# spectralDNS/mpiFFT4py

Hardware: AMD Instinct MI355X
Metric: 3D R2C+C2R pairs/sec, 1024^3 fp64 slab (higher is better)
Workload: dtype f64; 1 GPU; 1024^3 fp64 slab R2C forward+inverse, device-resident, 1 rank(s); gpus_visible=1

## Files before the change

### mpifft4py_amd/csrc/core.hip

```cpp
#include <algorithm>
#include <cstdarg>
#include <type_traits>
#include <cstdio>
#include <cstdlib>
#include <map>
#include <mutex>
#include <unordered_map>
#include <tuple>
#include "mfft_internal.h"
#include "fft_nlz.h"

namespace mfft {

static thread_local std::string g_err;

int set_error(int code, const char* fmt, ...) {
  char buf[1024];
  va_list ap;
  va_start(ap, fmt);
  vsnprintf(buf, sizeof buf, fmt, ap);
  va_end(ap);
  g_err = buf;
  return code;
}
const char* last_error() { return g_err.c_str(); }

std::vector<KernelEntry>& kernel_registry() {
  static std::vector<KernelEntry> reg;
  return reg;
}

constexpr int OP_BITS = 5, BUILD_BITS = 3, FAMILY_BITS = 6;
static_assert(2 * (unsigned)Op::TopFlag <= (1u << OP_BITS) && (unsigned)Op::Band < (unsigned)Op::Limited, "Op does not fit its key field");
static_assert((unsigned)Build::Last < (1u << BUILD_BITS), "Build does not fit its key field");
static_assert((unsigned)FAM_NLZ < (1u << FAMILY_BITS), "Family does not fit its key field");
static uint64_t kernel_key(int family, int n, int prec, int inv, Op op, Build build) {
  uint64_t k = (unsigned)n;
  k = k << FAMILY_BITS | (uint64_t)family;
  k = k << OP_BITS | (uint64_t)op;
  k = k << BUILD_BITS | (uint64_t)build;
  return k << 2 | (uint64_t)(inv << 1 | prec);
}

const KernelEntry* find_kernel(int family, int n, int prec, int inv, Op op, Build build) {
  static std::unordered_map<uint64_t, const KernelEntry*> index;
  static std::once_flag once;
  std::call_once(once, [] {
// ... 328 lines not shown
    P.bhat = static_cast<const cx<T>*>(bhat);
    P.n = a.n;
  }
  P.in = a.in;
  P.out = a.out;
  P.tw = static_cast<const cx<T>*>(tw);
  P.rtw = static_cast<const cx<T>*>(rtw);
  P.in_stride = a.in_stride;
  P.out_stride = a.out_stride;
  P.nrows = a.nrows;
  P.valid = a.valid > 0 ? a.valid : a.n / 2 + 1;
  P.scale = (T)a.scale;
  if constexpr (std::is_same<PT, RealParams<T>>::value) set_zsplit(P, a.zs);
  return launch_rows(e, P, a.nrows, e->tile, s);
}

static int c2r_mlds_mode() {
  static const int m = getenv("MFFT_C2R_MLDS") ? atoi(getenv("MFFT_C2R_MLDS")) : 1;
  return m;
}
static bool c2r_mlds_take(int n, int prec, bool limited) {
  const int m = c2r_mlds_mode();
  if (m <= 0) return false;
  if (m == 2) return true;
  if (m == 3) return limited;
  const int c = n / 2;
  if (c == 1000 || c == 2000) return prec == MFFT_SINGLE;
  if (c == 1536) return limited && prec == MFFT_SINGLE;
  if (c == 2048) return !limited && prec == MFFT_DOUBLE;
  return true;
// ... 6 lines not shown
    if (const KernelEntry* em = find_kernel(fam, a.n, a.prec, 1, op, Build::LdsMirrors)) e = em;
  const int64_t real_stride = fam == FAM_R2C ? a.in_stride : a.out_stride;
  if (a.zs.nchunk && (!e || real_stride % 2 != 0)) return set_error(MFFT_ERR_UNSUPPORTED, "no z-chunked real kernel of length %d", a.n);
  if (!e && limited) return set_error(MFFT_ERR_UNSUPPORTED, "no column-limited real kernel of length %d", a.n);
  if (!e || (real_stride % 2 != 0 && !limited)) {
    const bool r2c = fam == FAM_R2C;
    const bool half = a.n % 2 == 0 && a.n >= 4 && real_stride % 2 == 0;
    e = find_chirpz(half ? (r2c ? FAM_R2CZH : FAM_C2RZH) : (r2c ? FAM_R2CZ : FAM_C2RZ), half ? a.n / 2 : a.n, a.prec, r2c ? 0 : 1);
    if (!e && !big_length_ok(a.n)) return set_error(MFFT_ERR_UNSUPPORTED, "no kernel for a real transform of length %d", a.n);
  } else if (real_stride % 2 != 0) {
    return set_error(MFFT_ERR_UNSUPPORTED, "real row stride %lld must be even", (long long)real_stride);
  }
  *out = e;
  return 0;
}
static int launch_real(int fam, const RealArgs& a, hipStream_t s) {
  const KernelEntry* e = nullptr;
  MFFT_TRY(select_real(fam, a, &e));
  if (!e) return big_real(fam == FAM_C2R, a, s);
  void *tw = nullptr, *rtw = nullptr, *chirp = nullptr, *bhat = nullptr;
  MFFT_TRY(prepare_kernel(e, &tw));
  if (e->family != fam) {
    const bool half = e->family == FAM_R2CZH || e->family == FAM_C2RZH;
    MFFT_TRY(chirpz_tables(half ? a.n / 2 : a.n, e->n, a.prec, &chirp, &bhat));
    if (half) MFFT_TRY(real_twiddles(a.n, a.prec, &rtw));
    return by_prec(a.prec, [&](auto t) { return launch_real_t<decltype(t), RealParamsZ<decltype(t)>>(e, a, tw, rtw, s, chirp, bhat); });
  }
  MFFT_TRY(real_twiddles(a.n, a.prec, &rtw));
  return by_prec(a.prec, [&](auto t) { return launch_real_t<decltype(t)>(e, a, tw, rtw, s); });
}

int launch_r2c(const RealArgs& a, hipStream_t s) { return launch_real(FAM_R2C, a, s); }
// ... 208 lines not shown
```

### mpifft4py_amd/csrc/fft_kernels.h

```cpp
#pragma once
#include "fft_core.h"

#if defined(__HIPCC__)
#define MFFT_D __device__ __forceinline__
#define MFFT_BARRIER() __syncthreads()
#if defined(__HIP_DEVICE_COMPILE__)
#define MFFT_OPAQUE(x) asm volatile("" : "+v"(x))
#else
#define MFFT_OPAQUE(x) ((void)0)
#endif
template <class S, bool ORIGIN = false> MFFT_D int row_thread_index(int tid) {
  int j = tid % S::TPT;
  if constexpr (::mfft::launder_plan<S>()) {
#if MFFT_LAUNDER_MODE == 1
    MFFT_OPAQUE(j);
#elif MFFT_LAUNDER_MODE == 4
    if constexpr (ORIGIN) MFFT_OPAQUE(j);
#endif
  }
  return j;
}
#else
#define MFFT_OPAQUE(x) ((void)0)
template <class S, bool ORIGIN = false> inline int row_thread_index(int tid) { return tid % S::TPT; }
// ... 114 lines not shown
};

template <typename T>
struct RealParams {
  const void* in;
  void* out;
  const cx<T>* tw;
  const cx<T>* rtw;
  i64 in_stride, out_stride;
  i64 nrows;
  int valid;
  T scale;
  ZSplit zs;
  i64 row0;
};

template <int PD> MFFT_HD int padpos(int pos) {
  if constexpr (PD > 0) return pos + pos / PD;
  else return pos;
}
template <int N, int PD> constexpr int padded_len() { return PD > 0 ? N + N / PD + 1 : N; }
template <int PD> struct PadSlot {
  MFFT_D int operator()(int pos) const { return padpos<PD>(pos); }
};

template <typename T, class Slot>
struct XchFull {
  cx<T>* buf;
  Slot slot;
  template <class S, int P>
// ... 447 lines not shown
      for (int k = 0; k < S::E; ++k) {
        cx<T> x = scale(v[k], P.scale);
        x = INV ? swapri(x) : x;
        if constexpr (CHUNK && !INV) {
          bool ok;
          const i64 o = zsplit_off(P.zs, crow, j + k * S::TPT, &ok);
          if (ok) P.out[o] = x;
        } else {
          op[j + k * S::TPT] = x;
        }
      }
    }
  }
};

template <class S, typename T, int ROWS, bool TWLDS, bool LIMIT = false, bool CHUNK = false, bool SPLIT = false, bool WP = false>
struct R2CFft {
  typedef typename RowXch<SPLIT, T, PadSlot<S::R(0)>>::elem XE;
  static constexpr int M = S::N;
  static constexpr int RPW = WP ? 64 / S::TPT : 1;
  static_assert(!WP || (S::TPT < 64 && 64 % S::TPT != 0 && ROWS % (64 / S::TPT) == 0), "wave-packed rows: whole waves of rows");
  static constexpr int THREADS = WP ? ROWS / RPW * 64 : S::TPT * ROWS;
  static constexpr int PD = S::R(0);
  static constexpr int PLEN = padded_len<M, PD>();
  static constexpr int TW_BYTES = TWLDS ? (int)(S::TW * sizeof(cx<T>)) : 0;
  static constexpr int XCH_BYTES = (int)(PLEN * ROWS * sizeof(XE));
  static constexpr int LDS_BYTES = TW_BYTES + XCH_BYTES;

  static MFFT_D void body(const RealParams<T>& P, int bid, int tid, char* lds) {
    cx<T>* ltw = reinterpret_cast<cx<T>*>(lds);
    int rl, j, lane0 = 0;
    bool dup = false;
    if constexpr (WP) {
      const int lane = tid & 63;
      int lr = lane / S::TPT;
      dup = lr >= RPW;
      if (dup) lr = RPW - 1;
      lane0 = lr * S::TPT;
      j = dup ? lane - RPW * S::TPT : lane - lane0;
#if MFFT_LAUNDER_MODE == 1
      if constexpr (S::E % 15 == 0) MFFT_OPAQUE(j);
#endif
      rl = (tid >> 6) * RPW + lr;
    } else {
      rl = tid / S::TPT;
      j = row_thread_index<S>(tid);
    }
    XE* xch = reinterpret_cast<XE*>(lds + TW_BYTES) + rl * PLEN;
    const i64 row = (i64)bid * ROWS + rl;
    const bool inrange = row < P.nrows;
    const bool active = inrange && !dup;
    const cx<T>* ip =
        reinterpret_cast<const cx<T>*>(static_cast<const T*>(P.in) + (inrange ? row : P.nrows - 1) * P.in_stride);
    cx<T>* op = static_cast<cx<T>*>(P.out) + row * P.out_stride;

    cx<T> v[S::E];
#pragma unroll
    for (int k = 0; k < S::E; ++k) v[k] = ip[j + k * S::TPT];
    if constexpr (TWLDS && S::NP > 1) {
      stage_twiddles<S, T>(ltw, P.tw, tid, THREADS);
      MFFT_BARRIER();
    }
    typename RowXch<SPLIT, T, PadSlot<PD>>::type xc{xch, PadSlot<PD>{}};
    if constexpr (TWLDS) run_passes<S, 0, T>(v, j, (const cx<T>*)ltw, xc);
    else run_passes<S, 0, T>(v, j, P.tw, xc);

    const T half = (T)0.5;
    auto put = [&](int pos, cx<T> val) {
      if constexpr (CHUNK) {
// ... 5 lines not shown
      }
    };
    auto emit_w = [&](int pos, cx<T> zk, cx<T> zpartner, cx<T> w) {
      if (pos == 0) {
        put(0, mk<T>((zk.x + zk.y) * P.scale, (T)0));
        if (!LIMIT || M < P.valid) put(M, mk<T>((zk.x - zk.y) * P.scale, (T)0));
      } else if (!LIMIT || pos < P.valid) {
        const cx<T> zm = conj(zpartner);
        const cx<T> e = scale(zk + zm, half);
        const cx<T> o = mul_mi(scale(zk - zm, half));
        put(pos, scale(e + w * o, P.scale));
      }
    };
    auto emit = [&](int pos, cx<T> zk, cx<T> zpartner) { emit_w(pos, zk, zpartner, P.rtw[pos]); };
    constexpr bool SHFL = WP || (S::TPT <= 64 && (64 % S::TPT) == 0);
    if constexpr (SHFL) {
      const int src = WP ? lane0 + (j == 0 ? 0 : S::TPT - j) : (tid & 63) - j + ((S::TPT - j) & (S::TPT - 1));
      constexpr bool RTW_EARLY = S::E * (int)sizeof(cx<T>) <= 128;
      cx<T> rt[RTW_EARLY ? S::E : 1];
      if constexpr (RTW_EARLY) {
#pragma unroll
        for (int k = 0; k < S::E; ++k) rt[k] = P.rtw[j + k * S::TPT];
      }
#pragma unroll
      for (int k = 0; k < S::E; ++k) {
        const cx<T> give = v[S::E - 1 - k];
        cx<T> pm = mk<T>(wave_shfl(give.x, src), wave_shfl(give.y, src));
        if (j == 0) pm = v[(S::E - k) % S::E];
        if constexpr (RTW_EARLY) {
          if (active) emit_w(j + k * S::TPT, v[k], pm, rt[k]);
        } else
// ... 32 lines not shown
#pragma unroll
      for (int k = 0; k < S::E; ++k) xc.put(j + k * S::TPT, v[k]);
      MFFT_BARRIER();
      if (active) {
#pragma unroll
        for (int k = 0; k < S::E; ++k) {
          const int pos = j + k * S::TPT;
          emit(pos, v[k], xc.get(pos == 0 ? 0 : M - pos));
        }
      }
    }
  }
};

template <class S, typename T, int ROWS, bool TWLDS, bool LIMIT = false, bool CHUNK = false, bool SPLIT = false, bool WP = false,
          bool MLDS = false>
struct C2RFft {
  typedef typename RowXch<SPLIT, T, PadSlot<S::R(0)>>::elem XE;
  static constexpr int M = S::N;
  static constexpr int RPW = WP ? 64 / S::TPT : 1;
  static_assert(!WP || (S::TPT < 64 && 64 % S::TPT != 0 && ROWS % (64 / S::TPT) == 0), "wave-packed rows: whole waves of rows");
  static constexpr int THREADS = WP ? ROWS / RPW * 64 : S::TPT * ROWS;
  static constexpr int PD = S::R(0);
  static constexpr int PLEN = padded_len<M, PD>();
  static constexpr int TW_BYTES = TWLDS ? (int)(S::TW * sizeof(cx<T>)) : 0;
  static constexpr int XCH_BYTES = S::NP > 1 ? (int)(PLEN * ROWS * sizeof(XE)) : 0;
  static constexpr int LDS_BYTES = TW_BYTES + XCH_BYTES;

  static MFFT_D void body(const RealParams<T>& P, int bid, int tid, char* lds) {
    cx<T>* ltw = reinterpret_cast<cx<T>*>(lds);
    int rl, j, lane0 = 0;
    bool dup = false;
    if constexpr (WP) {
      const int lane = tid & 63;
      int lr = lane / S::TPT;
      dup = lr >= RPW;
      if (dup) lr = RPW - 1;
      lane0 = lr * S::TPT;
      j = dup ? lane - RPW * S::TPT : lane - lane0;
      if constexpr (S::E % 15 == 0) MFFT_OPAQUE(j);
      rl = (tid >> 6) * RPW + lr;
    } else {
      rl = tid / S::TPT;
      j = row_thread_index<S, true>(tid);
    }
    XE* xch = reinterpret_cast<XE*>(lds + TW_BYTES) + rl * PLEN;
    const i64 row = (i64)bid * ROWS + rl;
    const bool inrange = row < P.nrows;
    const bool active = inrange && !dup;
    const cx<T>* ip = static_cast<const cx<T>*>(P.in) + (inrange ? row : P.nrows - 1) * P.in_stride;
    cx<T>* op = reinterpret_cast<cx<T>*>(static_cast<T*>(P.out) + row * P.out_stride);

    const i64 crow = P.row0 + (inrange ? row : P.nrows - 1);
    auto bin = [&](int pos) -> cx<T> {
      if constexpr (CHUNK) {
        bool ok;
        const i64 o = zsplit_off(P.zs, crow, pos, &ok);
        const cx<T> x = static_cast<const cx<T>*>(P.in)[ok ? o : (i64)0];
        if constexpr (sizeof(T) == 4) return keep_bits(x, ok);
        else return ok ? x : mk<T>((T)0, (T)0);
      } else {
        return ip[pos];
      }
    };
    cx<T> v[S::E];
    constexpr bool SHFL = WP || (S::TPT <= 64 && (64 % S::TPT) == 0);
    if constexpr (SHFL) {
      static_assert(S::E % 2 == 0, "register pairing needs an even number of values per thread");
#pragma unroll
      for (int k = 0; k < S::E; ++k) {
        const int pos = j + k * S::TPT;
        if constexpr (LIMIT && sizeof(T) == 4) {
          const bool ok = pos < P.valid;
          v[k] = keep_bits(bin(ok ? pos : 0), ok);
        } else if constexpr (LIMIT) {
          v[k] = mk<T>((T)0, (T)0);
          if (pos < P.valid) v[k] = bin(pos);
        } else {
          v[k] = bin(pos);
        }
      }
      cx<T> carry = mk<T>((T)0, (T)0);
// ... 20 lines not shown
        if constexpr (WP || S::E % 7 != 0) {
          pm1 = mk<T>(wave_shfl(give1.x, src), wave_shfl(give1.y, src));
          pm2 = mk<T>(wave_shfl(give2.x, src), wave_shfl(give2.y, src));
        } else {
          pm1 = mk<T>(WAVE_SHFL_DIRECT(give1.x, src), WAVE_SHFL_DIRECT(give1.y, src));
          pm2 = mk<T>(WAVE_SHFL_DIRECT(give2.x, src), WAVE_SHFL_DIRECT(give2.y, src));
        }
        carry = b;
        v[k] = prepass(a, pm1, j + k * S::TPT);
        v[kp] = prepass(b, pm2, j + kp * S::TPT);
        if constexpr (S::E % 15 == 0) {
          if (k % 3 == 2) MFFT_SCHED_FENCE();
        }
      }
    } else if constexpr (MLDS && S::NP > 1) {
#pragma unroll
      for (int k = 0; k < S::E; ++k) {
        const int pos = j + k * S::TPT;
        if constexpr (LIMIT) {
          const bool ok = pos < P.valid;
          v[k] = keep_bits(bin(ok ? pos : 0), ok);
        } else {
          v[k] = bin(pos);
        }
      }
      cx<T> xM = mk<T>((T)0, (T)0);
      if (j == 0 && (!LIMIT || M < P.valid)) xM = bin(M);
      auto prepass = [&](cx<T> xk, cx<T> pm, int pos) {
        cx<T> xm = conj(pm);
        if (pos == 0) {
// ... 85 lines not shown
```

### mpifft4py_amd/csrc/mfft_internal.h

```cpp
#pragma once
#include <hip/hip_runtime.h>
#include <stdint.h>
#include <string>
#include <vector>
#include "../../include/mpifft4py_amd.h"
#include "registry.h"

namespace mfft {

int set_error(int code, const char* fmt, ...) __attribute__((format(printf, 2, 3)));
const char* last_error();

#define MFFT_HIP(call)                                                                   \
  do {                                                                                   \
    hipError_t e_ = (call);                                                              \
    if (e_ != hipSuccess)                                                                \
      return ::mfft::set_error(MFFT_ERR_HIP, "%s failed: %s (%s:%d)", #call,             \
                               hipGetErrorString(e_), __FILE__, __LINE__);               \
  } while (0)

#define MFFT_TRY(call)                  \
  do {                                  \
    int rc_ = (call);                   \
    if (rc_ != 0) return rc_;           \
// ... 53 lines not shown
  int64_t in_stride = 0, out_stride = 0, nrows = 0;
  double scale = 1.0;
  ZSplitArgs zs;
};
int launch_row(const RowArgs& a, hipStream_t s);

struct RealArgs {
  const void* in = nullptr;
  void* out = nullptr;
  int n = 0;
  int prec = MFFT_DOUBLE;
  int64_t in_stride = 0, out_stride = 0, nrows = 0;
  double scale = 1.0;
  int valid = 0;
  ZSplitArgs zs;
};
int launch_r2c(const RealArgs& a, hipStream_t s);
int launch_c2r(const RealArgs& a, hipStream_t s);

struct NlzArgs {
  const void* a[3] = {nullptr, nullptr, nullptr};
  const void* b[3] = {nullptr, nullptr, nullptr};
  void* out[3] = {nullptr, nullptr, nullptr};
  int n = 0;
  int prec = MFFT_DOUBLE;
  int64_t in_stride = 0, out_stride = 0, nrows = 0;
  int valid = 0;
  int valid_in = 0;
  double scale = 1.0;
};
bool nlz_supported(int64_t n, int prec);
int launch_nlz(const NlzArgs& a, hipStream_t s);

// ... 32 lines not shown
```

### mpifft4py_amd/csrc/plan_create.hip

```cpp
#include "plan_impl.h"

using namespace mfft;

#ifndef MFFT_DEFAULT_COMM_CUS
#define MFFT_DEFAULT_COMM_CUS 0
#endif

mfft_plan_s::~mfft_plan_s() {
  for (Buf* b : {&work[0], &work[1], &work[2], &work3, &nlw[0], &nlw[1], &nlx, &nly, &nlr, &pcomp})
    if (b->p) (void)(b->arena ? wfree(b->p) : dev_free(b->p));
  if (mask) (void)hipFree(mask);
  if (band_tiles) (void)hipFree(band_tiles);
  for (auto& t : timers) {
    for (auto& e : t.pending) { (void)hipEventDestroy(e.first); (void)hipEventDestroy(e.second); }
    for (auto& e : t.pool) { (void)hipEventDestroy(e.first); (void)hipEventDestroy(e.second); }
  }
  drop_graphs();
  for (hipEvent_t e : ev_compute) (void)hipEventDestroy(e);
  for (hipEvent_t e : ev_comm) (void)hipEventDestroy(e);
  for (hipEvent_t e : ev2_compute) (void)hipEventDestroy(e);
  for (hipEvent_t e : ev2_comm) (void)hipEventDestroy(e);
  if (cstream) { big_release_stream(cstream); (void)hipStreamDestroy(cstream); }
  if (stream) { big_release_stream(stream); (void)hipStreamDestroy(stream); }
}
// ... 287 lines not shown
  if (!p || !key || !value) return set_error(MFFT_ERR_INVALID, "null argument");
  const std::string k(key);
  if (k == "pruned_route") *value = p->band_ok ? (p->band_allzero ? 2 : 1) : 0;
  else if (k == "local_band") *value = p->lband_ok ? 1 : 0;
  else if (k == "comm_cus") *value = p->comm_cus;
  else if (k == "kz_slices") *value = p->nslice;
  else if (k == "row_batches") *value = p->nbatch;
  else if (k == "zfuse") *value = p->zfuse ? 1 : 0;
  else if (k == "ranks") *value = p->P;
  else if (k == "complex_pitch") *value = p->pitched() ? p->Zp : 0;
  else if (k == "complex_pitch_native") *value = p->nat_pitch() ? 1 : 0;
  else if (k == "nonlinear_fused_none") *value = p->nonlinear_fusable(MFFT_DEALIAS_NONE) ? 1 : 0;
  else if (k == "nonlinear_fused_2_3") *value = p->nonlinear_fusable(MFFT_DEALIAS_2_3) ? 1 : 0;
  else if (k == "nonlinear_fused_3_2") *value = p->nonlinear_fusable(MFFT_DEALIAS_3_2) ? 1 : 0;
  else if (k == "nonlinear_bytes") *value = (int64_t)(p->nlx.bytes + p->nly.bytes + p->nlr.bytes + p->nlw[0].bytes + p->nlw[1].bytes);
  else if (k == "plane_pad") *value = (p->P == 1 && p->d.decomp == MFFT_SLAB) ? p->p1_plane_pad() : 0;
  else return set_error(MFFT_ERR_INVALID, "mfft_plan_get_info: unknown key '%s'", key);
  return 0;
}

int mfft_plan_timing(mfft_plan_t p, int enable) {
  if (!p) return set_error(MFFT_ERR_INVALID, "null plan");
  p->timing = enable != 0;
  return 0;
}

int mfft_plan_timing_reset(mfft_plan_t p) {
  if (!p) return set_error(MFFT_ERR_INVALID, "null plan");
  MFFT_TRY(p->collect_timing());
  for (auto& t : p->timers) {
// ... 24 lines not shown
```

### mpifft4py_amd/csrc/plan_impl.h

```cpp
#pragma once
#include <algorithm>
#include <cmath>
#include <cstdlib>
#include <cstring>
#include <memory>
#include <string>
#include "comm.h"
#include "mfft_internal.h"

#ifndef MFFT_P1_XPAD_DEFAULT
#define MFFT_P1_XPAD_DEFAULT 0
#endif

namespace mfft {

inline bool env_on(const char* name) {
  const char* e = getenv(name);
  return e && atoi(e) != 0;
}
inline long env_int(const char* name, long dflt) {
  const char* e = getenv(name);
  return e ? atol(e) : dflt;
}

// ... 273 lines not shown
    return 0;
  }
  int exchange_piece(const char* name, int which, bool forward, int piece, const void* send, void* recv, hipEvent_t done) {
    MFFT_TRY(stage_on(cstream, name, 0, [&] {
      Sched sc;
      MFFT_TRY(piece_sched(which, forward, piece, &sc));
      return run_sched(sc, send, recv, cstream);
    }));
    MFFT_HIP(hipEventRecord(done, cstream));
    return 0;
  }
  int npieces() const { return nbatch > 1 ? nbatch : nslice > 1 ? nslice : 1; }
  int piece_sched(int which, bool forward, int piece, Sched* out) const;

  bool fwd_out_of_place(size_t cbytes);
  int slab_forward(const void* u, void* fu);
  int slab_backward(const void* fu, void* u, bool masked);
  int slab_backward_pruned(const void* fu, void* u);
  int slab_forward_pipelined(const void* u, void* fu);
  int slab_backward_pipelined(const void* src, void* u, bool pruned = false);
  int slab_forward_rows(const void* u, void* fu);
  int slab_backward_rows(const void* src, void* u, bool pruned = false);

  int pack_z(const void* Z, void* S, int64_t rows, int64_t nf, bool unpack);
  int pencil_forward_pipelined_x(const void* u, void* fu);
  int pencil_backward_pipelined_x(const void* src, void* u);
  int pencil_forward_pipelined_y(const void* u, void* fu);
  int pencil_backward_pipelined_y(const void* src, void* u);
  int pencil_forward(const void* u, void* fu);
  int pencil_backward(const void* fu, void* u, bool masked);
// ... 97 lines not shown
```

### mpifft4py_amd/csrc/plan_sched.hip

```cpp
#include "plan_impl.h"
#include "relay_plan.h"

using namespace mfft;

namespace {

std::vector<Chunk> pencil_chunks(int64_t n, int size) {
  std::vector<Chunk> c(size);
  const int64_t q = n / size, r = n % size;
  for (int i = 0; i < size; ++i) c[i] = Chunk{q + ((r == 1 && i == size - 1) ? 1 : 0), q * i};
  return c;
}

void compute_dims(int n, int* p1, int* p2) {
  int best1 = n, best2 = 1;
  for (int a = 1; a * a <= n; ++a)
    if (n % a == 0) {
      best1 = n / a;
      best2 = a;
    }
  *p1 = best1;
  *p2 = best2;
}

// ... 188 lines not shown
  p->Nf = p->r2c ? p->N2 / 2 + 1 : p->N2;
  p->es = elem_bytes(p->prec, true);
  p->rs = p->r2c ? elem_bytes(p->prec, false) : p->es;
  const double ps = desc->padsize > 0 ? desc->padsize : 1.5;
  p->d.padsize = ps;
  p->M0 = (int64_t)(ps * p->N0);
  p->M1 = (int64_t)(ps * p->N1);
  p->M2 = (int64_t)(ps * p->N2);
  p->Mf = p->r2c ? (int64_t)(ps * p->N2) / 2 + 1 : p->M2;
  p->world.resize(p->P);
  for (int i = 0; i < p->P; ++i) p->world[i] = i;
  p->xpad_on = !env_on("MFFT_NO_XPAD");
  p->xpass_inplace = env_on("MFFT_XPASS_INPLACE");
  p->p1_xpad_lines = (int)env_int("MFFT_P1_XPAD", p->p1_xpad_lines);
  p->zpitch_on = !env_on("MFFT_NO_ZPITCH");
  if (getenv("MFFT_PAD_ALIGN")) p->pad_align = env_on("MFFT_PAD_ALIGN") ? 1 : 0;
  p->pad_align_inv = (int)env_int("MFFT_PAD_ALIGN_INV", p->pad_align_inv);
  const int P = p->P;
  if (p->r2c && p->N2 % 2) return set_error(MFFT_ERR_UNSUPPORTED, "odd N[2]=%lld is not supported for R2C", (long long)p->N2);
  p->Zp = 0;
  if (desc->decomp == MFFT_SLAB) {
    if (p->N0 % P || p->N1 % P) return set_error(MFFT_ERR_INVALID, "N[0]=%lld and N[1]=%lld must be divisible by the number of ranks %d", (long long)p->N0, (long long)p->N1, P);
    p->Np0 = p->N0 / P;
    p->Np1 = p->N1 / P;
    if (P > 1 && desc->pipeline < 0) {
      p->nbatch = (int)std::min<int64_t>(-(int64_t)desc->pipeline, p->Np0);
    } else if (P > 1) {
      const int want = desc->pipeline > 0 ? desc->pipeline : 4;
      const int64_t unit = 16;
      const int64_t per = (p->Nf / want) / unit * unit;
// ... 130 lines not shown
```

### mpifft4py_amd/csrc/plan_slab.hip

```cpp
#include "plan_impl.h"

using namespace mfft;

#ifndef MFFT_FWD_OOP_DEFAULT
#define MFFT_FWD_OOP_DEFAULT 0
#endif

bool mfft_plan_s::fwd_out_of_place(size_t cbytes) {
  static const int mode = (int)env_int("MFFT_FWD_OOP", MFFT_FWD_OOP_DEFAULT);
  if (mode <= 0) return false;
  if (work[0].bytes >= cbytes) return true;
  size_t fr = 0, tot = 0;
  if (hipMemGetInfo(&fr, &tot) != hipSuccess) { (void)hipGetLastError(); return false; }
  return cbytes <= fr / 4;
}

int mfft_plan_s::slab_forward(const void* u, void* fu) {
  const double Cb = (double)(N0 * Np1 * Nf) * es;
  const double Rb = (double)(Np0 * N1 * N2) * rs;
  if (P == 1) {
    const int64_t Z = Zc();
    if (const int64_t xpad = p1_plane_pad()) {
      MFFT_TRY(stage("fwd_z", Rb + Cb, [&] { return z_forward(u, fu, N0 * N1, N2, Z); }));
      const int64_t pl = N1 * Z + xpad;
      MFFT_TRY(ensure(work[0], (size_t)(N0 * pl) * es));
      void* A = work[0].p;
      MFFT_TRY(stage("fwd_y", 2 * Cb, [&] { return col(fu, A, N1, false, N0, Nf, N1 * Z, plain(Z), pl, plain(Z)); }));
      MFFT_TRY(stage("fwd_x", 2 * Cb, [&] { return col(A, fu, N0, false, 1, N1 * Z, 0, plain(pl), 0, plain(N1 * Z)); }));
      return 0;
    }
    MFFT_TRY(stage("fwd_z", Rb + Cb, [&] { return z_forward(u, fu, N0 * N1, N2, Z); }));
    if (fwd_out_of_place((size_t)Cb)) {
      MFFT_TRY(ensure(work[0], (size_t)(N0 * N1 * Z) * es));
      void* A = work[0].p;
// ... 67 lines not shown
    return col_band(fu, Aw, N0, Np1, a2, Nf, plain(Np1 * Nf), ap, plain(Np1 * ap), bx);
  }));
  MFFT_TRY(stage("bwd_a2a", 0, [&] { return exchange_equal(world, Aw, Bw, (size_t)(Np0 * Np1 * ap) * es); }));
  MFFT_TRY(stage("bwd_y", 2 * Cb * keep2, [&] {
    return col(Bw, Aw, N1, true, Np0, a2, Np1 * ap, two_level(Np1, Np0 * Np1 * ap, ap), N1 * ap, plain(ap));
  }));
  MFFT_TRY(stage("bwd_z", Rb + Cb * keep2, [&] { return c2r_rows(Aw, u, Np0 * N1, N2, ap, N2, 1.0 / (double)N2, (int)a2); }));
  return 0;
}

int mfft_plan_s::slab_backward(const void* fu, void* u, bool masked) {
  const double Cb = (double)(N0 * Np1 * Nf) * es;
  const double Rb = (double)(Np0 * N1 * N2) * rs;
  const void* src = fu;
  MaskScope mask_scope{this};
  if (masked && band_ok && prune_enabled()) {
    MFFT_TRY(require_mask());
    return slab_backward_pruned(fu, u);
  }
  if (masked) {
    bool fused = false;
    MFFT_TRY(fuse_mask(fu, (P == 1 && p1_plane_pad()) ? N1 : N0, &fused));
    if (!fused) {
      void* m = nullptr;
      MFFT_TRY(stage("bwd_mask", 2 * Cb, [&] { return apply_mask_copy(fu, &m); }));
      src = m;
    }
  }
  const int64_t Z = P == 1 ? Zc() : Nf;
  const size_t cb = (size_t)(Np0 * N1 * Z) * es;
// ... 186 lines not shown
```

### mpifft4py_amd/csrc/registry.h

```cpp
#pragma once
#include <hip/hip_runtime.h>
#include <cstring>
#include <type_traits>
#include <vector>
#include "fft_kernels.h"
#include "fft_chirpz.h"
#include "fft_col3.h"
#include "twiddle.h"
#include "plans.h"

namespace mfft {

enum Family {
  FAM_COL = 0, FAM_ROW = 1, FAM_R2C = 2, FAM_C2R = 3,
  FAM_COLZ = 4, FAM_ROWZ = 5, FAM_R2CZ = 6, FAM_C2RZ = 7,
  FAM_R2CZH = 8, FAM_C2RZH = 9,
  FAM_NLZ = 10
};

enum class Op : unsigned {
  Plain = 0,
  PadLoad = 1,
  TruncStore = 2,
  MaskLoad = 3,
  Band = 4,
  Limited = 8,
  ZChunk = 16,
  TopFlag = ZChunk
};
constexpr Op operator|(Op a, Op b) { return (Op)((unsigned)a | (unsigned)b); }
constexpr bool has(Op a, Op flag) { return ((unsigned)a & (unsigned)flag) != 0; }
enum class Build : unsigned {
  Default = 0,
  NonTemporal,
  YTile,
  Col3,
  Col3NT,
  Col3Thirds,
  LdsMirrors,
  Nlz3,
  Last = Nlz3
};

// ... 310 lines not shown
  if (sizeof(T) == 8 && FAM != 2 && S::N == 500 && S::E == 20) return 768 / threads;
  if (sizeof(T) == 8 && FAM == 0 && (S::N == 800 || S::N == 2000) && S::E == 20) return 1024 / threads;
  return 0;
}

#ifndef MFFT_C2R_MLDS
#define MFFT_C2R_MLDS 1
#endif
template <class S, typename T> constexpr bool c2r_mlds_candidate() {
  if (!MFFT_C2R_MLDS || S::NP < 2 || c2r_wave_packed<S, T>() || (S::TPT <= 64 && 64 % S::TPT == 0)) return false;
  if (S::E == 12 && (S::N == 1152 || S::N == 2304)) return true;
  if (S::E == 12 && (S::N == 432 || S::N == 864 || S::N == 1728 || S::N == 3456 || S::N == 288 || S::N == 576)) return true;
  if ((S::E == 12 && (S::N == 1536 || S::N == 3072)) || (S::E == 16 && (S::N == 2048 || S::N == 4096))) return true;
  if (S::E == 20 && (S::N == 400 || S::N == 500 || S::N == 800 || S::N == 1000 || S::N == 2000)) return true;
  return false;
}
template <class S, typename T>
void register_rows(const char* name) {
  auto& reg = kernel_registry();
  constexpr int R = row_rows<S, T>();
  constexpr int WO = row_occ_wgs<S, T>(S::TPT * R);
  constexpr int WO5 = row_occ_r5<S, T, 0>(S::TPT * R) ? row_occ_r5<S, T, 0>(S::TPT * R) : WO;
  constexpr bool WPC = c2r_wave_packed<S, T>();
  constexpr bool WPR = r2c_wave_packed<S, T>();
  constexpr int WOC = (MFFT_ROW_OCC_C2R && (WPC || (S::TPT <= 64 && 64 % S::TPT == 0))) ? row_occ_wgs<S, T>(c2r_threads<S, T>()) : 0;
  constexpr int WOV = (MFFT_ROW_OCC_C2R && sizeof(T) == 8 && S::E == 20 && S::N >= 160 && c2r_threads<S, T>() <= 256)
                          ? 512 / c2r_threads<S, T>() : WOC;
  constexpr bool RT = row_twlds<S, T>();
  constexpr bool SP = row_split<S, T>();
  constexpr int RC = c2r_rows<S, T>();
// ... 24 lines not shown
  row(tag<false>, tag<Op::Plain>, tag<WO5>);
  row(tag<true>, tag<Op::Plain>, tag<WO5>);
  r2c(tag<Op::Plain>, tag<WOR5>);
  c2r(tag<Op::Plain>, tag<false>, tag<(WOC5 ? WOC5 : WOC)>);
  row(tag<false>, tag<Op::ZChunk>, tag<WO>);
  row(tag<true>, tag<Op::ZChunk>, tag<WO>);
  r2c(tag<Op::ZChunk>, tag<WOR>);
  c2r(tag<Op::ZChunk>, tag<false>, tag<WOV>);
  if constexpr (S::N % 3 == 0 && S::N >= 6) {
    r2c(tag<Op::Limited>, tag<WOR>);
    r2c(tag<LZ>, tag<WOR>);
    c2r(tag<LZ>, tag<false>, tag<WOV>);
  }
  if constexpr (S::N >= 4)
    c2r(tag<Op::Limited>, tag<false>, tag<WOV>);
  if constexpr (c2r_mlds_candidate<S, T>()) {
    c2r(tag<Op::Plain>, tag<true>, tag<WOC>);
    c2r(tag<Op::ZChunk>, tag<true>, tag<WOV>);
    c2r(tag<Op::Limited>, tag<true>, tag<WOV>);
    if constexpr (S::N % 3 == 0 && S::N >= 6) c2r(tag<LZ>, tag<true>, tag<WOV>);
  }
}

template <class S, typename T> constexpr int colz_cols() {
  constexpr int c = col_wide_small<S, T>() > 0 ? 128 / (int)sizeof(cx<T>) : col_cols<S, T>(), v = col_vec<S, T>();
  return (col_split<S, T>() && S::TPT * (c / v) > 512 && c / 2 >= v && c / 2 >= 64 / (int)sizeof(cx<T>) &&
          (long long)S::N * (c / 2) * (int)sizeof(cx<T>) <= 131072 && S::TPT * (c / 2 / v) >= 64) ? c / 2 : c;
}
template <class S, typename T> constexpr bool colz_split() {
  return S::NP > 1 && (long long)S::N * colz_cols<S, T>() * (int)sizeof(cx<T>) > 131072;
// ... 57 lines not shown
```

Before: 50.29 pairs/s.

## Route 1024^3 fp64 slab through split-last pairing: complex x/y passes then paired real z

Adds a split-last slab route for single-rank real transforms. The real input is treated as N2/2 complex values per line, and the complex x and y column passes run first on that half-size data. A new pair-row R2C/C2R kernel then handles the last axis by processing each Hermitian-conjugate row pair (kx,ky) with (-kx,-ky) together through LDS, which recovers the real-to-complex spectrum. The aim is to avoid running the x/y passes on the larger N2/2+1 complex spectrum and to cut memory traffic, at the cost of an extra padded work buffer and a new kernel family. It is enabled by default only for 1024^3 double precision.

```diff
diff --git a/mpifft4py_amd/csrc/core.hip b/mpifft4py_amd/csrc/core.hip
--- a/mpifft4py_amd/csrc/core.hip
+++ b/mpifft4py_amd/csrc/core.hip
@@ -30,7 +30,7 @@
   return reg;
 }
 
-constexpr int OP_BITS = 5, BUILD_BITS = 3, FAMILY_BITS = 6;
+constexpr int OP_BITS = 6, BUILD_BITS = 3, FAMILY_BITS = 6;
 static_assert(2 * (unsigned)Op::TopFlag <= (1u << OP_BITS) && (unsigned)Op::Band < (unsigned)Op::Limited, "Op does not fit its key field");
 static_assert((unsigned)Build::Last < (1u << BUILD_BITS), "Build does not fit its key field");
 static_assert((unsigned)FAM_NLZ < (1u << FAMILY_BITS), "Family does not fit its key field");
@@ -389,6 +389,25 @@
   if constexpr (std::is_same<PT, RealParams<T>>::value) set_zsplit(P, a.zs);
   return launch_rows(e, P, a.nrows, e->tile, s);
 }
+template <typename T>
+static int launch_pair_t(const KernelEntry* e, const RealArgs& a, void* tw, void* rtw, hipStream_t s) {
+  RealPairParams<T> P;
+  P.in = a.in;
+  P.out = a.out;
+  P.tw = static_cast<const cx<T>*>(tw);
+  P.rtw = static_cast<const cx<T>*>(rtw);
+  P.in_stride = a.in_stride;
+  P.out_stride = a.out_stride;
+  P.nrows = (int64_t)(a.pair_n0 / 2 + 1) * a.pair_n1;
+  P.valid = a.n / 2 + 1;
+  P.scale = (T)a.scale;
+  set_zsplit(P, a.zs);
+  P.pn0 = a.pair_n0;
+  P.pn1 = a.pair_n1;
+  P.p_rplane = a.pair_rplane;
+  P.p_cplane = a.pair_cplane;
+  return launch_rows(e, P, P.nrows, e->tile / 2, s);
+}
 
 static int c2r_mlds_mode() {
   static const int m = getenv("MFFT_C2R_MLDS") ? atoi(getenv("MFFT_C2R_MLDS")) : 1;
@@ -425,8 +444,22 @@
   *out = e;
   return 0;
 }
+bool pair_rows_supported(int64_t n, int prec) {
+  return n >= 2 && n < 65536 && find_kernel(FAM_R2C, (int)n, prec, 0, Op::PairRows) && find_kernel(FAM_C2R, (int)n, prec, 1, Op::PairRows);
+}
 static int launch_real(int fam, const RealArgs& a, hipStream_t s) {
   const KernelEntry* e = nullptr;
+  if (a.pair_n0 > 0) {
+    e = find_kernel(fam, a.n, a.prec, fam == FAM_C2R ? 1 : 0, Op::PairRows);
+    const int64_t real_stride = fam == FAM_R2C ? a.in_stride : a.out_stride;
+    if (!e || a.zs.nchunk || a.valid > 0 || real_stride % 2 != 0 || a.pair_rplane % 2 != 0 ||
+        a.nrows != (int64_t)a.pair_n0 * a.pair_n1 || a.nrows >= (int64_t)1 << 31)
+      return set_error(MFFT_ERR_UNSUPPORTED, "no pair-row real kernel of length %d for this layout", a.n);
+    void *tw = nullptr, *rtw = nullptr;
+    MFFT_TRY(prepare_kernel(e, &tw));
+    MFFT_TRY(real_twiddles(a.n, a.prec, &rtw));
+    return by_prec(a.prec, [&](auto t) { return launch_pair_t<decltype(t)>(e, a, tw, rtw, s); });
+  }
   MFFT_TRY(select_real(fam, a, &e));
   if (!e) return big_real(fam == FAM_C2R, a, s);
   void *tw = nullptr, *rtw = nullptr, *chirp = nullptr, *bhat = nullptr;
diff --git a/mpifft4py_amd/csrc/fft_kernels.h b/mpifft4py_amd/csrc/fft_kernels.h
--- a/mpifft4py_amd/csrc/fft_kernels.h
+++ b/mpifft4py_amd/csrc/fft_kernels.h
@@ -1,4 +1,5 @@
 #pragma once
+#include <type_traits>
 #include "fft_core.h"
 
 #if defined(__HIPCC__)
@@ -152,6 +153,32 @@
   ZSplit zs;
   i64 row0;
 };
+template <typename T>
+struct RealPairParams : RealParams<T> {
+  int pn0, pn1;
+  i64 p_rplane, p_cplane;
+};
+
+struct PairRow {
+  i64 real_off, cplx_off;
+  bool live;
+};
+template <typename T>
+MFFT_D PairRow pair_row(const RealPairParams<T>& P, i64 q, int side, i64 real_pitch, i64 cplx_pitch) {
+  const bool inrange = q < P.nrows;
+  if (!inrange) q = P.nrows - 1;
+  const unsigned n0 = (unsigned)P.pn0, n1 = (unsigned)P.pn1;
+  const unsigned kx = (unsigned)q / n1, ky = (unsigned)q - kx * n1;
+  const unsigned px = kx ? n0 - kx : 0u, py = ky ? n1 - ky : 0u;
+  bool live = inrange && !(px == kx && ky > py);
+  if (side && px == kx && py == ky) live = false;
+  const unsigned x = side ? px : kx, y = side ? py : ky;
+  PairRow r;
+  r.real_off = (i64)x * P.p_rplane + (i64)y * real_pitch;
+  r.cplx_off = (i64)x * P.p_cplane + (i64)y * cplx_pitch;
+  r.live = live;
+  return r;
+}
 
 template <int PD> MFFT_HD int padpos(int pos) {
   if constexpr (PD > 0) return pos + pos / PD;
@@ -629,9 +656,12 @@
   }
 };
 
-template <class S, typename T, int ROWS, bool TWLDS, bool LIMIT = false, bool CHUNK = false, bool SPLIT = false, bool WP = false>
+template <class S, typename T, int ROWS, bool TWLDS, bool LIMIT = false, bool CHUNK = false, bool SPLIT = false, bool WP = false,
+          bool PAIR = false>
 struct R2CFft {
   typedef typename RowXch<SPLIT, T, PadSlot<S::R(0)>>::elem XE;
+  static_assert(!PAIR || (!LIMIT && !CHUNK && !SPLIT && !WP && ROWS % 2 == 0 && S::NP > 1), "pair rows: plain dense kernels, whole pairs");
+  typedef typename std::conditional<PAIR, RealPairParams<T>, RealParams<T>>::type Params;
   static constexpr int M = S::N;
   static constexpr int RPW = WP ? 64 / S::TPT : 1;
   static_assert(!WP || (S::TPT < 64 && 64 % S::TPT != 0 && ROWS % (64 / S::TPT) == 0), "wave-packed rows: whole waves of rows");
@@ -642,7 +672,7 @@
   static constexpr int XCH_BYTES = (int)(PLEN * ROWS * sizeof(XE));
   static constexpr int LDS_BYTES = TW_BYTES + XCH_BYTES;
 
-  static MFFT_D void body(const RealParams<T>& P, int bid, int tid, char* lds) {
+  static MFFT_D void body(const Params& P, int bid, int tid, char* lds) {
     cx<T>* ltw = reinterpret_cast<cx<T>*>(lds);
     int rl, j, lane0 = 0;
     bool dup = false;
@@ -663,11 +693,13 @@
     }
     XE* xch = reinterpret_cast<XE*>(lds + TW_BYTES) + rl * PLEN;
     const i64 row = (i64)bid * ROWS + rl;
-    const bool inrange = row < P.nrows;
-    const bool active = inrange && !dup;
+    PairRow pr{};
+    if constexpr (PAIR) pr = pair_row<T>(P, (i64)bid * (ROWS / 2) + (rl >> 1), rl & 1, P.in_stride, P.out_stride);
+    const bool inrange = PAIR ? true : row < P.nrows;
+    const bool active = PAIR ? pr.live : inrange && !dup;
     const cx<T>* ip =
-        reinterpret_cast<const cx<T>*>(static_cast<const T*>(P.in) + (inrange ? row : P.nrows - 1) * P.in_stride);
-    cx<T>* op = static_cast<cx<T>*>(P.out) + row * P.out_stride;
+        reinterpret_cast<const cx<T>*>(static_cast<const T*>(P.in) + (PAIR ? pr.real_off : (inrange ? row : P.nrows - 1) * P.in_stride));
+    cx<T>* op = static_cast<cx<T>*>(P.out) + (PAIR ? pr.cplx_off : row * P.out_stride);
 
     cx<T> v[S::E];
 #pragma unroll
@@ -703,7 +735,37 @@
     };
     auto emit = [&](int pos, cx<T> zk, cx<T> zpartner) { emit_w(pos, zk, zpartner, P.rtw[pos]); };
     constexpr bool SHFL = WP || (S::TPT <= 64 && (64 % S::TPT) == 0);
-    if constexpr (SHFL) {
+    if constexpr (PAIR) {
+      const XE* pxch = reinterpret_cast<const XE*>(lds + TW_BYTES) + (rl ^ 1) * PLEN;
+      constexpr bool RTW_EARLY = S::E * (int)sizeof(cx<T>) <= 128;
+      cx<T> rt[RTW_EARLY ? S::E : 1];
+      if constexpr (RTW_EARLY) {
+#pragma unroll
+        for (int k = 0; k < S::E; ++k) rt[k] = P.rtw[j + k * S::TPT];
+      }
+      MFFT_BARRIER();
+#pragma unroll
+      for (int k = 0; k < S::E; ++k) xc.put(j + k * S::TPT, v[k]);
+      MFFT_BARRIER();
+      if (active) {
+#pragma unroll
+        for (int k = 0; k < S::E; ++k) {
+          const int pos = j + k * S::TPT;
+          const cx<T> zm = conj(pxch[padpos<PD>(pos == 0 ? 0 : M - pos)]);
+          const cx<T> e = scale(v[k] + zm, half);
+          const cx<T> o = mul_mi(scale(v[k] - zm, half));
+          if (pos == 0) {
+            put(0, scale(e + o, P.scale));
+            put(M, scale(e - o, P.scale));
+          } else {
+            cx<T> w;
+            if constexpr (RTW_EARLY) w = rt[k];
+            else w = P.rtw[pos];
+            put(pos, scale(e + w * o, P.scale));
+          }
+        }
+      }
+    } else if constexpr (SHFL) {
       const int src = WP ? lane0 + (j == 0 ? 0 : S::TPT - j) : (tid & 63) - j + ((S::TPT - j) & (S::TPT - 1));
       constexpr bool RTW_EARLY = S::E * (int)sizeof(cx<T>) <= 128;
       cx<T> rt[RTW_EARLY ? S::E : 1];
@@ -766,9 +828,11 @@
 };
 
 template <class S, typename T, int ROWS, bool TWLDS, bool LIMIT = false, bool CHUNK = false, bool SPLIT = false, bool WP = false,
-          bool MLDS = false>
+          bool MLDS = false, bool PAIR = false>
 struct C2RFft {
   typedef typename RowXch<SPLIT, T, PadSlot<S::R(0)>>::elem XE;
+  static_assert(!PAIR || (!LIMIT && !CHUNK && !SPLIT && !WP && !MLDS && ROWS % 2 == 0 && S::NP > 1), "pair rows: plain dense kernels, whole pairs");
+  typedef typename std::conditional<PAIR, RealPairParams<T>, RealParams<T>>::type Params;
   static constexpr int M = S::N;
   static constexpr int RPW = WP ? 64 / S::TPT : 1;
   static_assert(!WP || (S::TPT < 64 && 64 % S::TPT != 0 && ROWS % (64 / S::TPT) == 0), "wave-packed rows: whole waves of rows");
@@ -779,7 +843,7 @@
   static constexpr int XCH_BYTES = S::NP > 1 ? (int)(PLEN * ROWS * sizeof(XE)) : 0;
   static constexpr int LDS_BYTES = TW_BYTES + XCH_BYTES;
 
-  static MFFT_D void body(const RealParams<T>& P, int bid, int tid, char* lds) {
+  static MFFT_D void body(const Params& P, int bid, int tid, char* lds) {
     cx<T>* ltw = reinterpret_cast<cx<T>*>(lds);
     int rl, j, lane0 = 0;
     bool dup = false;
@@ -798,10 +862,12 @@
     }
     XE* xch = reinterpret_cast<XE*>(lds + TW_BYTES) + rl * PLEN;
     const i64 row = (i64)bid * ROWS + rl;
-    const bool inrange = row < P.nrows;
-    const bool active = inrange && !dup;
-    const cx<T>* ip = static_cast<const cx<T>*>(P.in) + (inrange ? row : P.nrows - 1) * P.in_stride;
-    cx<T>* op = reinterpret_cast<cx<T>*>(static_cast<T*>(P.out) + row * P.out_stride);
+    PairRow pr{};
+    if constexpr (PAIR) pr = pair_row<T>(P, (i64)bid * (ROWS / 2) + (rl >> 1), rl & 1, P.out_stride, P.in_stride);
+    const bool inrange = PAIR ? true : row < P.nrows;
+    const bool active = PAIR ? pr.live : inrange && !dup;
+    const cx<T>* ip = static_cast<const cx<T>*>(P.in) + (PAIR ? pr.cplx_off : (inrange ? row : P.nrows - 1) * P.in_stride);
+    cx<T>* op = reinterpret_cast<cx<T>*>(static_cast<T*>(P.out) + (PAIR ? pr.real_off : row * P.out_stride));
 
     const i64 crow = P.row0 + (inrange ? row : P.nrows - 1);
     auto bin = [&](int pos) -> cx<T> {
@@ -817,7 +883,33 @@
     };
     cx<T> v[S::E];
     constexpr bool SHFL = WP || (S::TPT <= 64 && (64 % S::TPT) == 0);
-    if constexpr (SHFL) {
+    if constexpr (PAIR) {
+      static_assert(PD > 0, "slot padpos(M) exists only in padded rows: PLEN = M + M / PD + 1");
+#pragma unroll
+      for (int k = 0; k < S::E; ++k) v[k] = ip[j + k * S::TPT];
+      cx<T> xM = mk<T>((T)0, (T)0);
+      if (j == 0) xM = ip[M];
+      const XE* pxch = reinterpret_cast<const XE*>(lds + TW_BYTES) + (rl ^ 1) * PLEN;
+#pragma unroll
+      for (int k = 0; k < S::E; ++k) xch[padpos<PD>(j + k * S::TPT)] = v[k];
+      if (j == 0) xch[padpos<PD>(M)] = xM;
+      MFFT_BARRIER();
+      const T half = (T)0.5;
+#pragma unroll
+      for (int k = 0; k < S::E; ++k) {
+        const int pos = j + k * S::TPT;
+        cx<T> xk = v[k];
+        cx<T> xm = conj(pxch[padpos<PD>(M - pos)]);
+        if (pos == 0) {
+          xk = scale(xk + conj(pxch[padpos<PD>(0)]), half);
+          xm = scale(xM + xm, half);
+        }
+        const cx<T> e = xk + xm;
+        const cx<T> dd = xk - xm;
+        v[k] = swapri(e + mul_pi(dd * conj(P.rtw[pos])));
+      }
+      MFFT_BARRIER();
+    } else if constexpr (SHFL) {
       static_assert(S::E % 2 == 0, "register pairing needs an even number of values per thread");
 #pragma unroll
       for (int k = 0; k < S::E; ++k) {
@@ -868,6 +960,7 @@
         }
       }
     } else if constexpr (MLDS && S::NP > 1) {
+      static_assert(PD > 0, "slot padpos(M) exists only in padded rows: PLEN = M + M / PD + 1");
 #pragma unroll
       for (int k = 0; k < S::E; ++k) {
         const int pos = j + k * S::TPT;
diff --git a/mpifft4py_amd/csrc/mfft_internal.h b/mpifft4py_amd/csrc/mfft_internal.h
--- a/mpifft4py_amd/csrc/mfft_internal.h
+++ b/mpifft4py_amd/csrc/mfft_internal.h
@@ -91,9 +91,12 @@
   double scale = 1.0;
   int valid = 0;
   ZSplitArgs zs;
+  int pair_n0 = 0, pair_n1 = 0;
+  int64_t pair_rplane = 0, pair_cplane = 0;
 };
 int launch_r2c(const RealArgs& a, hipStream_t s);
 int launch_c2r(const RealArgs& a, hipStream_t s);
+bool pair_rows_supported(int64_t n, int prec);
 
 struct NlzArgs {
   const void* a[3] = {nullptr, nullptr, nullptr};
diff --git a/mpifft4py_amd/csrc/plan_create.hip b/mpifft4py_amd/csrc/plan_create.hip
--- a/mpifft4py_amd/csrc/plan_create.hip
+++ b/mpifft4py_amd/csrc/plan_create.hip
@@ -325,6 +325,7 @@
   else if (k == "nonlinear_fused_2_3") *value = p->nonlinear_fusable(MFFT_DEALIAS_2_3) ? 1 : 0;
   else if (k == "nonlinear_fused_3_2") *value = p->nonlinear_fusable(MFFT_DEALIAS_3_2) ? 1 : 0;
   else if (k == "nonlinear_bytes") *value = (int64_t)(p->nlx.bytes + p->nly.bytes + p->nlr.bytes + p->nlw[0].bytes + p->nlw[1].bytes);
+  else if (k == "split_last") *value = p->split_last_route() ? 1 : 0;
   else if (k == "plane_pad") *value = (p->P == 1 && p->d.decomp == MFFT_SLAB) ? p->p1_plane_pad() : 0;
   else return set_error(MFFT_ERR_INVALID, "mfft_plan_get_info: unknown key '%s'", key);
   return 0;
diff --git a/mpifft4py_amd/csrc/plan_impl.h b/mpifft4py_amd/csrc/plan_impl.h
--- a/mpifft4py_amd/csrc/plan_impl.h
+++ b/mpifft4py_amd/csrc/plan_impl.h
@@ -311,6 +311,13 @@
   int piece_sched(int which, bool forward, int piece, Sched* out) const;
 
   bool fwd_out_of_place(size_t cbytes);
+  int split_last = -1;
+  int split_last_fit = -1;
+  int64_t split_last_pad() const { return plane_pad(N1 * (N2 / 2)); }
+  bool split_last_eligible() const;
+  bool split_last_route();
+  int slab_forward_split_last(const void* u, void* fu);
+  int slab_backward_split_last(const void* fu, void* u);
   int slab_forward(const void* u, void* fu);
   int slab_backward(const void* fu, void* u, bool masked);
   int slab_backward_pruned(const void* fu, void* u);
diff --git a/mpifft4py_amd/csrc/plan_sched.hip b/mpifft4py_amd/csrc/plan_sched.hip
--- a/mpifft4py_amd/csrc/plan_sched.hip
+++ b/mpifft4py_amd/csrc/plan_sched.hip
@@ -226,6 +226,7 @@
   p->xpass_inplace = env_on("MFFT_XPASS_INPLACE");
   p->p1_xpad_lines = (int)env_int("MFFT_P1_XPAD", p->p1_xpad_lines);
   p->zpitch_on = !env_on("MFFT_NO_ZPITCH");
+  if (getenv("MFFT_SPLIT_LAST")) p->split_last = env_on("MFFT_SPLIT_LAST") ? 1 : 0;
   if (getenv("MFFT_PAD_ALIGN")) p->pad_align = env_on("MFFT_PAD_ALIGN") ? 1 : 0;
   p->pad_align_inv = (int)env_int("MFFT_PAD_ALIGN_INV", p->pad_align_inv);
   const int P = p->P;
diff --git a/mpifft4py_amd/csrc/plan_slab.hip b/mpifft4py_amd/csrc/plan_slab.hip
--- a/mpifft4py_amd/csrc/plan_slab.hip
+++ b/mpifft4py_amd/csrc/plan_slab.hip
@@ -15,9 +15,54 @@
   return cbytes <= fr / 4;
 }
 
+bool mfft_plan_s::split_last_eligible() const {
+  if (d.decomp != MFFT_SLAB || P != 1 || !r2c || nat_pitch() || d.line2d || d.drop_nyquist || split_last == 0) return false;
+  if (N0 < 2 || N1 < 2 || N2 % 2 || !pair_rows_supported(N2, prec)) return false;
+  if (split_last > 0) return true;
+  return prec == MFFT_DOUBLE && N0 == 1024 && N1 == 1024 && N2 == 1024;
+}
+bool mfft_plan_s::split_last_route() {
+  if (!split_last_eligible()) return false;
+  if (split_last_fit < 0) {
+    const size_t need = (size_t)(N0 * (N1 * (N2 / 2) + split_last_pad())) * es;
+    size_t fr = 0, tot = 0;
+    if (work[0].bytes >= need) split_last_fit = 1;
+    else if (hipMemGetInfo(&fr, &tot) != hipSuccess) { (void)hipGetLastError(); split_last_fit = 0; }
+    else split_last_fit = need <= fr / 4 ? 1 : 0;
+  }
+  return split_last_fit == 1;
+}
+int mfft_plan_s::slab_forward_split_last(const void* u, void* fu) {
+  const int64_t M = N2 / 2, pl = N1 * M + split_last_pad();
+  const double Wb = (double)(N0 * N1 * M) * es;
+  MFFT_TRY(ensure(work[0], (size_t)(N0 * pl) * es));
+  void* W = work[0].p;
+  MFFT_TRY(stage("fwd_x", 2 * Wb, [&] { return col(u, W, N0, false, 1, N1 * M, 0, plain(N1 * M), 0, plain(pl)); }));
+  MFFT_TRY(stage("fwd_y", 2 * Wb, [&] { return col(W, W, N1, false, N0, M, pl, plain(M), pl, plain(M)); }));
+  return stage("fwd_z", Wb + (double)(N0 * N1 * Nf) * es, [&] {
+    RealArgs a = real_args(W, fu, N0 * N1, N2, N2, Nf, 1.0);
+    a.pair_n0 = (int)N0; a.pair_n1 = (int)N1; a.pair_rplane = 2 * pl; a.pair_cplane = N1 * Nf;
+    return mfft::launch_r2c(a, stream);
+  });
+}
+int mfft_plan_s::slab_backward_split_last(const void* fu, void* u) {
+  const int64_t M = N2 / 2, pl = N1 * M + split_last_pad();
+  const double Wb = (double)(N0 * N1 * M) * es;
+  MFFT_TRY(ensure(work[0], (size_t)(N0 * pl) * es));
+  void* W = work[0].p;
+  MFFT_TRY(stage("bwd_z", Wb + (double)(N0 * N1 * Nf) * es, [&] {
+    RealArgs a = real_args(fu, W, N0 * N1, N2, Nf, N2, 1.0 / (double)N2);
+    a.pair_n0 = (int)N0; a.pair_n1 = (int)N1; a.pair_rplane = 2 * pl; a.pair_cplane = N1 * Nf;
+    return mfft::launch_c2r(a, stream);
+  }));
+  MFFT_TRY(stage("bwd_y", 2 * Wb, [&] { return col(W, W, N1, true, N0, M, pl, plain(M), pl, plain(M)); }));
+  return stage("bwd_x", 2 * Wb, [&] { return col(W, u, N0, true, 1, N1 * M, 0, plain(pl), 0, plain(N1 * M)); });
+}
+
 int mfft_plan_s::slab_forward(const void* u, void* fu) {
   const double Cb = (double)(N0 * Np1 * Nf) * es;
   const double Rb = (double)(Np0 * N1 * N2) * rs;
+  if (P == 1 && split_last_route()) return slab_forward_split_last(u, fu);
   if (P == 1) {
     const int64_t Z = Zc();
     if (const int64_t xpad = p1_plane_pad()) {
@@ -115,6 +160,7 @@
   const double Rb = (double)(Np0 * N1 * N2) * rs;
   const void* src = fu;
   MaskScope mask_scope{this};
+  if (!masked && P == 1 && split_last_route()) return slab_backward_split_last(fu, u);
   if (masked && band_ok && prune_enabled()) {
     MFFT_TRY(require_mask());
     return slab_backward_pruned(fu, u);
diff --git a/mpifft4py_amd/csrc/registry.h b/mpifft4py_amd/csrc/registry.h
--- a/mpifft4py_amd/csrc/registry.h
+++ b/mpifft4py_amd/csrc/registry.h
@@ -26,7 +26,8 @@
   Band = 4,
   Limited = 8,
   ZChunk = 16,
-  TopFlag = ZChunk
+  PairRows = 32,
+  TopFlag = PairRows
 };
 constexpr Op operator|(Op a, Op b) { return (Op)((unsigned)a | (unsigned)b); }
 constexpr bool has(Op a, Op flag) { return ((unsigned)a & (unsigned)flag) != 0; }
@@ -367,6 +368,13 @@
   if ((S::E == 12 && (S::N == 1536 || S::N == 3072)) || (S::E == 16 && (S::N == 2048 || S::N == 4096))) return true;
   if (S::E == 20 && (S::N == 400 || S::N == 500 || S::N == 800 || S::N == 1000 || S::N == 2000)) return true;
   return false;
+}
+template <class S, typename T> constexpr bool pair_rows_plan() {
+  return sizeof(T) == 8 && S::NP > 1 && (S::N == 32 || S::N == 128 || S::N == 512 || S::N == 1024);
+}
+template <class S, typename T> constexpr int pair_rows() {
+  constexpr int r = row_rows_n<S, T, false>();
+  return r < 2 ? 2 : r;
 }
 template <class S, typename T>
 void register_rows(const char* name) {
@@ -421,6 +429,14 @@
   }
   if constexpr (S::N >= 4)
     c2r(tag<Op::Limited>, tag<false>, tag<WOV>);
+  if constexpr (pair_rows_plan<S, T>()) {
+    constexpr int RP = pair_rows<S, T>();
+    constexpr bool TP = S::N <= 512;
+    reg.push_back(make_entry<R2CFft<S, T, RP, TP, false, false, false, false, true>, RealPairParams<T>, S, T>(
+        FAM_R2C, 2 * S::N, 0, Op::PairRows, Build::Default, RP, name));
+    reg.push_back(make_entry<C2RFft<S, T, RP, TP, false, false, false, false, false, true>, RealPairParams<T>, S, T>(
+        FAM_C2R, 2 * S::N, 1, Op::PairRows, Build::Default, RP, name));
+  }
   if constexpr (c2r_mlds_candidate<S, T>()) {
     c2r(tag<Op::Plain>, tag<true>, tag<WOC>);
     c2r(tag<Op::ZChunk>, tag<true>, tag<WOV>);
```

Result: faster. 51.25 pairs/s, median of 6 (+1.9%).
